# tudelft-iv/CCVPE

Measured on AMD Instinct MI355X. Metric: image-pairs/sec, higher is better.
Workload: dtype f32

## Files before the change

### ccvpe_amd/_lib.py

```python
import ctypes
import os
import subprocess

import torch

_HERE = os.path.dirname(os.path.abspath(__file__))
LIB_PATH = os.environ.get("CCVPE_LIB") or os.path.join(_HERE, "libccvpe_hip.so")
CSRC_DIR = os.path.join(_HERE, "csrc")

c_float_p = ctypes.c_void_p
c_int = ctypes.c_int
c_float = ctypes.c_float
c_void_p = ctypes.c_void_p


class ConvDesc(ctypes.Structure):
    _fields_ = [
        ("src0", c_void_p), ("src1", c_void_p), ("gate", c_void_p), ("w", c_void_p),
        ("scale", c_void_p), ("shift", c_void_p), ("residual", c_void_p), ("dst", c_void_p),
        ("c0", c_int), ("ld0", c_int), ("c1", c_int), ("ld1", c_int),
        ("batch", c_int), ("in_h", c_int), ("in_w", c_int),
        ("kh", c_int), ("kw", c_int), ("stride", c_int), ("pad", c_int),
        ("n", c_int), ("kpad", c_int), ("ldd", c_int), ("ldres", c_int),
        ("act", c_int), ("out_mode", c_int),
# ... 35 lines not shown
    "ccvpe_tail512_f32": (c_int, [ctypes.POINTER(TailDesc), c_void_p]),
    "ccvpe_tail512_bf16": (c_int, [ctypes.POINTER(TailDesc), c_void_p]),
    "ccvpe_conv_igemm_f32": (c_int, [ctypes.POINTER(ConvDesc), c_void_p]),
    "ccvpe_conv_igemm_splitk_floats": (c_int, [ctypes.POINTER(ConvDesc), c_int]),
    "ccvpe_conv_igemm_route": (c_int, [ctypes.POINTER(ConvDesc), c_int, c_int]),
    "ccvpe_set_narrow_kernels": (c_int, [c_int]),
    "ccvpe_set_pw_ring_kernels": (c_int, [c_int]),
    "ccvpe_set_mbconv_plane_kernels": (c_int, [c_int]),
    "ccvpe_mbconv_front_route": (c_int, [c_int] * 8),
    "ccvpe_mbconv_band_plan": (c_int, [c_int] * 7),
    "ccvpe_conv3x3_variant": (c_int, [ctypes.POINTER(ConvDesc), c_int]),
    "ccvpe_set_match_mfma": (c_int, [c_int]),
    "ccvpe_set_pwn_kernels": (c_int, [c_int]),
    "ccvpe_conv3x3_wino_ok": (c_int, [ctypes.POINTER(ConvDesc)]),
    "ccvpe_conv3x3_wino_f32": (c_int, [ctypes.POINTER(ConvDesc), c_void_p]),
    "ccvpe_conv3x3_match1_ok": (c_int, [ctypes.POINTER(ConvDesc), c_int, c_int]),
    "ccvpe_conv3x3_match1_bf16": (c_int, [ctypes.POINTER(ConvDesc), c_int, c_void_p, c_int, c_int, c_int, c_int, c_int, c_void_p, c_void_p]),
    "ccvpe_conv_igemm_splitk_f32": (c_int, [ctypes.POINTER(ConvDesc), c_void_p, c_void_p]),
    "ccvpe_conv_igemm_splitk_bf16": (c_int, [ctypes.POINTER(ConvDesc), c_int, c_void_p, c_void_p]),
    "ccvpe_upconv3x3_f32": (c_int, [ctypes.POINTER(UpconvDesc), c_void_p]),
    "ccvpe_upconv3x3_bf16": (c_int, [ctypes.POINTER(UpconvDesc), c_void_p]),
    "ccvpe_upconv3x3_route": (c_int, [ctypes.POINTER(UpconvDesc), c_int]),
    "ccvpe_upconv3x3_s3_ok": (c_int, [ctypes.POINTER(UpconvDesc)]),
    "ccvpe_upconv3x3_s3_f32": (c_int, [ctypes.POINTER(UpconvDesc), c_void_p]),
    "ccvpe_upconv3x3_s3_form_ok": (c_int, [ctypes.POINTER(UpconvDesc), c_int]),
    "ccvpe_upconv3x3_s3_form_f32": (c_int, [ctypes.POINTER(UpconvDesc), c_int, c_void_p]),
    "ccvpe_set_s3_quad": (c_int, [c_int]),
    "ccvpe_stem_conv_f32": (c_int, [c_void_p] * 5 + [c_int] * 4 + [c_void_p]),
    "ccvpe_dwconv_nblk": (c_int, [c_int] * 4),
    "ccvpe_dwconv_f32": (c_int, [c_void_p] * 6 + [c_int] * 7 + [c_void_p]),
# ... 141 lines not shown
```

### ccvpe_amd/csrc/plan.hip

```cpp
#include <cstring>
#include <string>
#include <unordered_map>
#include <utility>
#include <vector>

#include "common.h"

namespace ccvpe {

enum : uint32_t { K_INT = 0, K_FLT = 1, K_NULL = 2, K_WEIGHTS = 3, K_WORKSPACE = 4, K_GRD = 5, K_SAT = 6, K_STREAM = 7, K_BLOB = 8 };

template <typename A> struct FromSlot {
  static A get(uint64_t v) { return (A)(int64_t)v; }
};
template <typename P> struct FromSlot<P*> {
  static P* get(uint64_t v) { return reinterpret_cast<P*>((uintptr_t)v); }
};
template <> struct FromSlot<float> {
  static float get(uint64_t v) { uint32_t b = (uint32_t)v; float f; std::memcpy(&f, &b, 4); return f; }
};
template <typename... A, size_t... I>
static int invoke_seq(int (*f)(A...), const uint64_t* v, std::index_sequence<I...>) { return f(FromSlot<A>::get(v[I])...); }
template <typename... A>
static int invoke(int (*f)(A...), const uint64_t* v, int n) {
  if (n != (int)sizeof...(A)) return fail(CCVPE_EINVAL, "plan: call has %d arguments, the entry point takes %d", n, (int)sizeof...(A));
  return invoke_seq(f, v, std::index_sequence_for<A...>{});
}
typedef int (*Invoker)(const uint64_t*, int);

#define CCVPE_REG(fn) {#fn, [](const uint64_t* v, int n) -> int { return invoke(fn, v, n); }}
static const std::unordered_map<std::string, Invoker>& registry() {
  static const std::unordered_map<std::string, Invoker> r = {
      CCVPE_REG(ccvpe_conv_igemm_f32), CCVPE_REG(ccvpe_conv_igemm_bf16), CCVPE_REG(ccvpe_conv_igemm_splitk_f32),
      CCVPE_REG(ccvpe_conv_igemm_splitk_bf16), CCVPE_REG(ccvpe_conv3x3_match1_bf16), CCVPE_REG(ccvpe_conv3x3_wino_f32),
      CCVPE_REG(ccvpe_upconv3x3_f32), CCVPE_REG(ccvpe_upconv3x3_bf16), CCVPE_REG(ccvpe_upconv3x3_s3_f32),
      CCVPE_REG(ccvpe_tail512_f32), CCVPE_REG(ccvpe_tail512_bf16), CCVPE_REG(ccvpe_stem_conv_f32), CCVPE_REG(ccvpe_stem_conv_bf16),
      CCVPE_REG(ccvpe_stem_dw_f32), CCVPE_REG(ccvpe_stem_dw_bf16),
      CCVPE_REG(ccvpe_dwconv_f32), CCVPE_REG(ccvpe_dwconv_bf16), CCVPE_REG(ccvpe_mbconv_front_f32), CCVPE_REG(ccvpe_mbconv_front_bf16),
      CCVPE_REG(ccvpe_se_gate_f32), CCVPE_REG(ccvpe_ground_descriptor_f32), CCVPE_REG(ccvpe_match_level_f32),
      CCVPE_REG(ccvpe_match_level_bf16), CCVPE_REG(ccvpe_head_conv3x3_f32), CCVPE_REG(ccvpe_head_conv3x3_bf16),
      CCVPE_REG(ccvpe_softmax_rows_f32), CCVPE_REG(ccvpe_softmax_apply_f32), CCVPE_REG(ccvpe_cast_bf16_f32), CCVPE_REG(ccvpe_eval_postprocess_f32),
  };
  return r;
}
#undef CCVPE_REG

struct Patch { uint32_t call, arg, kind; uint64_t off; };
struct BlobPatch { uint32_t blob, field, kind; uint64_t off; };
struct Call { Invoker fn; std::string name; uint32_t first, nargs, sid; int wait_on; };
// ... 245 lines not shown
```

### ccvpe_amd/csrc/upconv_s3.hip

```cpp
#include "conv_common.h"

namespace ccvpe {

struct UpS3Params {
  const float* src0;
  const float* src1;
  const void* w;
  const float* shift9;
  float* dst;
  int c0, ld0, c1, ld1;
  int H1, W1, batch;
  int N, Npad;
  int nb0, nb1, nst;
  int ldd, act;
  int tiles_n, tiles_total;
};

template <int MT, int NT, int WN, bool PAIR>
struct UpS3Geom {
  static constexpr int WM = 4 / WN;
  static constexpr int BM = 16 * MT * WM;
  static constexpr int BN = 16 * NT * WN;
  static constexpr int TH = BM / 16;
  static constexpr int HR = TH + 2, HCP = PAIR ? 26 : 18;
  static constexpr int ROW = 24;
  static constexpr int HALO_DW = HR * HCP * ROW, ASTG_DW = 2 * BM * ROW;
  static constexpr int U_DW = HALO_DW > ASTG_DW ? HALO_DW : ASTG_DW;
  static constexpr int W_INSTR = (BN * 6 + 63) / 64;
  static constexpr int WBUF_DW = W_INSTR * 256;
  static constexpr int LDS_BYTES = (U_DW + 2 * WBUF_DW) * 4;
};

__device__ __forceinline__ unsigned pk_bf16(float a, float b) {
  typedef __bf16 bf16x2_t __attribute__((ext_vector_type(2)));
  bf16x2_t v;
  v[0] = (__bf16)a;
  v[1] = (__bf16)b;
  return __builtin_bit_cast(unsigned, v);
}
__device__ __forceinline__ float bf_lo(unsigned p) { return __builtin_bit_cast(float, p << 16); }
__device__ __forceinline__ float bf_hi(unsigned p) { return __builtin_bit_cast(float, p & 0xffff0000u); }

typedef unsigned u32x2 __attribute__((ext_vector_type(2)));
__device__ __forceinline__ void split3(f32x4 v, u32x2& hi, u32x2& mid, u32x2& lo) {
#pragma unroll
  for (int h = 0; h < 2; ++h) {
    float a = v[2 * h], b = v[2 * h + 1];
    const unsigned ph = pk_bf16(a, b);
    a -= bf_lo(ph);
    b -= bf_hi(ph);
    const unsigned pm = pk_bf16(a, b);
    a -= bf_lo(pm);
    b -= bf_hi(pm);
    hi[h] = ph;
    mid[h] = pm;
    lo[h] = pk_bf16(a, b);
  }
}

template <int MT, int NT, int WN, bool PAIR>
__global__ __launch_bounds__(256, 2) void upconv_s3_kernel(const UpS3Params p) {
  using G = UpS3Geom<MT, NT, WN, PAIR>;
  constexpr int BM = G::BM, BN = G::BN, TH = G::TH, HR = G::HR, HCP = G::HCP, ROW = G::ROW;
  constexpr int HC = PAIR ? 20 : 18, HPX = HR * HC;
  constexpr int H_IT = (HPX * 4 + 255) / 256;
  constexpr int A_IT = BM / 64;
  constexpr int WQ = (G::W_INSTR + 3) / 4;

  extern __shared__ __attribute__((aligned(16))) float s3_sm[];
  float* Us = s3_sm;
  float* Ws = s3_sm + G::U_DW;

  const int tid = threadIdx.x;
// ... 37 lines not shown
      h_pix[it] = -1;
    }
  }
  f32x4 h_reg[H_IT];
  unsigned h_keep = 0;
  auto load_halo = [&](int chunk) {
    h_keep = 0;
#pragma unroll
    for (int it = 0; it < H_IT; ++it) {
      const int ch = chunk * 16 + h_sub[it] * 4;
      const bool ok = h_pix[it] >= 0 && ch < p.c0;
      h_reg[it] = *reinterpret_cast<const f32x4*>(reinterpret_cast<const char*>(p.src0) + (ok ? ((unsigned)h_pix[it] * (unsigned)ld0s + (unsigned)ch) * 4u : 0u));
      h_keep |= ok ? (1u << it) : 0u;
    }
  };
  auto store_planes = [&](float* at, f32x4 v) {
    u32x2 hi, mid, lo;
    split3(v, hi, mid, lo);
    *reinterpret_cast<u32x2*>(at) = hi;
    *reinterpret_cast<u32x2*>(at + 8) = mid;
    *reinterpret_cast<u32x2*>(at + 16) = lo;
  };
  auto store_halo = [&]() {
#pragma unroll
    for (int it = 0; it < H_IT; ++it)
      if (h_off[it] >= 0) store_planes(Us + h_off[it], keep_if(h_reg[it], (h_keep >> it) & 1u));
  };

  unsigned wvoff[WQ];
  {
    const int valid = min(BN, p.Npad - n0) * 6;
#pragma unroll
    for (int q = 0; q < WQ; ++q) wvoff[q] = (unsigned)min((wave + 4 * q) * 64 + lane, valid - 1) * 16u;
  }
  const unsigned ws_lds = (unsigned)(uintptr_t)(__attribute__((address_space(3))) float*)Ws;
  const size_t stage_bytes = (size_t)p.Npad * (ROW * 4);
  const char* wpar = reinterpret_cast<const char*>(p.w) + ((size_t)par * p.nst * p.Npad + n0) * (ROW * 4);
// ... 266 lines not shown
```

### ccvpe_amd/models.py

```python
import torch
import torch.nn as nn

from . import ops
from .synth import B0_BLOCKS, MODEL_SPECS, state_dict_spec

BN_EPS = 1e-3
SKIP_BLOCKS = (15, 10, 4, 2, 0)
MATCH_STRIDES = {"vigor": (64, 32, 16, 8, 4, 2),
                 "kitti": (128, 64, 32, 16, 8, 8),
                 "oxford": (64, 32, 16, 8, 4, 2)}


def window_offset(kind, channels, length):
    return int(channels / 2 - length / 2) if kind == "oxford" else 0


def _round_up(v, m):
    return (v + m - 1) // m * m


class _Holder(nn.Module):

    def forward(self, *a, **k):
        raise RuntimeError("parameter holder is not callable; use the owning CVM_* module")
# ... 32 lines not shown
    return _pad2(w.permute(0, 2, 3, 1).reshape(o, -1), dtype)


_WINO_G = ((1.0, 0.0, 0.0), (0.5, 0.5, 0.5), (0.5, -0.5, 0.5), (0.0, 0.0, 1.0))


def _pack_wino(w, dtype=torch.float32):
    if dtype != torch.float32:
        return None
    o, i = w.shape[0], w.shape[1]
    g = torch.tensor(_WINO_G, dtype=torch.float64, device=w.device)
    u = torch.einsum("ak,ockl,bl->oabc", g, w.to(torch.float64), g)
    out = torch.zeros((_round_up(o, 32), 4, 4, _round_up(i, 16)), dtype=torch.float64, device=w.device)
    out[:o, :, :, :i] = u
    return out.reshape(out.shape[0], -1).to(torch.float32).contiguous()


def _fold_bn(sd, p):
    scale = sd[p + ".weight"] / torch.sqrt(sd[p + ".running_var"] + BN_EPS)
    shift = sd[p + ".bias"] - sd[p + ".running_mean"] * scale
    return scale.contiguous(), shift.contiguous()


class _Obj(object):
    pass


def _pack_encoder(sd, p, dtype=torch.float32, fold_bn=True):
    fold = _fold_bn if fold_bn else (lambda _sd, _p: (None, None))
    e = _Obj()
# ... 37 lines not shown


OVERLAP_DECODERS_MAX_BATCH = 128


def _overlap_decoders(precision, batch=1):
    return _OVERLAP_ENV == "1" or (_OVERLAP_ENV == "auto" and precision == "bf16" and batch <= OVERLAP_DECODERS_MAX_BATCH)
FOLD_LEVELS = tuple(int(c) for c in __import__("os").environ.get("CCVPE_FOLD_LEVELS", "012345"))
FOLD_MIN_PIXELS = int(__import__("os").environ.get("CCVPE_FOLD_MIN_PIXELS", "2048"))
FUSE_TAIL = __import__("os").environ.get("CCVPE_FUSE_TAIL", "1") != "0"
SPLIT_TAIL = __import__("os").environ.get("CCVPE_SPLIT_TAIL", "1") != "0"
WINO = __import__("os").environ.get("CCVPE_WINO", "1") != "0"
SPLIT3 = __import__("os").environ.get("CCVPE_SPLIT3", "1") != "0"
SPLIT3_TAIL = SPLIT3 and __import__("os").environ.get("CCVPE_SPLIT3_TAIL", "1") != "0"
SPLIT3_MIN_OK = 2
PACK_GRAPH = __import__("os").environ.get("CCVPE_PACK_GRAPH", "1") != "0"
PACK_GATHER = __import__("os").environ.get("CCVPE_PACK_GATHER", "1") != "0"
FUSE_MATCH = __import__("os").environ.get("CCVPE_FUSE_MATCH", "1") != "0"
FUSE_STEM = __import__("os").environ.get("CCVPE_FUSE_STEM", "1") != "0"
EVAL_TWO_STREAMS = __import__("os").environ.get("CCVPE_EVAL_TWO_STREAMS", "1") != "0"


def _tail_split(precision, x, cout):
    if x.dtype != torch.float32:
        return 0
    if precision == "bf16":
        return 1 if SPLIT_TAIL and cout == 1 else 0
    return 2 if SPLIT3 and SPLIT3_TAIL else 0


# ... 136 lines not shown
        lv.c, lv.ldo, lv.up_n = c, ldo, 4 * dc_out
        lv.up_w, lv.up_b = _pack_deconv(sd["deconv%d.weight" % lvl], sd["deconv%d.bias" % lvl],
                                        [(0, 1, c), (c, 0, 1)], ldo, dtype)
        lv.c0, lv.c1 = dc_out, c_in - dc_out
        lv.n_a = c_out
        if fold and j in FOLD_LEVELS:
            lv.fw, lv.fshift = _pack_upconv(sd["deconv%d.weight" % lvl], sd["deconv%d.bias" % lvl],
                                            [(0, 1, c), (c, 0, 1)], ldo, sd["conv%d.0.weight" % lvl],
                                            sd["conv%d.0.bias" % lvl], dtype)
            lv.fw3 = _pack_upconv_s3(lv.fw, ldo, lv.c1, dtype if base_dtype == torch.float32 else None)
        lv.w_a = _pack_conv(sd["conv%d.0.weight" % lvl], dtype)
        lv.b_a = sd["conv%d.0.bias" % lvl].contiguous()
        if lvl != 1:
            lv.w_b = _pack_conv(sd["conv%d.2.weight" % lvl], dtype)
            lv.u_b = _pack_wino(sd["conv%d.2.weight" % lvl], base_dtype) if fold else None
            lv.n_b = c_out
        else:
            lv.w_b = sd["conv1.2.weight"].permute(0, 2, 3, 1).contiguous()
        lv.b_b = sd["conv%d.2.bias" % lvl].contiguous()
        pk.loc.append(lv)
        dtype = base_dtype
        dc_in, dc_out, c_in, c_out = spec["ori"][j]
        ov = _Obj()
        if j == 0:
            c6 = dc_in - n_rot
            ov.k = pk.loc[0].ldo
            ov.k_algo = dc_in
            ov.up_w, ov.up_b = _pack_deconv(sd["deconv6_ori.weight"], sd["deconv6_ori.bias"],
                                            [(0, n_rot, c6), (c6 + 1, 0, n_rot)], pk.loc[0].ldo, dtype)
        else:
# ... 2 lines not shown
                                            [(0, 0, dc_in)], dc_in, dtype)
        ov.up_n = 4 * dc_out
        ov.c0, ov.c1 = dc_out, c_in - dc_out
        if fold and j in FOLD_LEVELS:
            cmap = [(0, n_rot, c6), (c6 + 1, 0, n_rot)] if j == 0 else [(0, 0, dc_in)]
            ov.fw, ov.fshift = _pack_upconv(sd["deconv%d_ori.weight" % lvl], sd["deconv%d_ori.bias" % lvl], cmap,
                                            ov.k, sd["conv%d_ori.0.weight" % lvl], sd["conv%d_ori.0.bias" % lvl],
                                            dtype)
            ov.fw3 = _pack_upconv_s3(ov.fw, ov.k, ov.c1, dtype)
        ov.w_a = _pack_conv(sd["conv%d_ori.0.weight" % lvl], dtype)
        ov.b_a = sd["conv%d_ori.0.bias" % lvl].contiguous()
        ov.n_a = c_out
        if lvl != 1:
            ov.w_b = _pack_conv(sd["conv%d_ori.2.weight" % lvl], dtype)
            ov.u_b = _pack_wino(sd["conv%d_ori.2.weight" % lvl], dtype) if fold else None
            ov.n_b = c_out
        else:
            ov.w_b = sd["conv1_ori.2.weight"].permute(0, 2, 3, 1).contiguous()
        ov.b_b = sd["conv%d_ori.2.bias" % lvl].contiguous()
        pk.ori.append(ov)
    pk.bwd = _pack_backward(sd, kind, pk) if (not fold and base_dtype == torch.float32) else None
    return pk


def _run_encoder(e, img, circular, multiscale, dtype=torch.float32):
    blk0 = e.blocks[0]
    stem_fused = (FUSE_STEM and not blk0.expand and blk0.k == 3 and blk0.s == 1 and blk0.mid == 32
                  and ops.stem_dw_supported(img.shape[2], img.shape[3], circular) > 0)
    x = None if stem_fused else ops.stem_conv(img, e.stem_w, e.stem_scale, e.stem_shift, circular, out_dtype=dtype)
    feats = []
# ... 20 lines not shown
        if multiscale:
            feats.append(x)
    b, h, w, _ = x.shape
    f = ops.conv_igemm(x, 320, e.w_head, 1280, batch=b, in_h=h, in_w=w, scale=e.head_scale,
                       shift=e.head_shift, act=ops.ACT_SWISH)
    return f, feats


def _double_conv(lv, up, skip, batch, hw):
    y = ops.conv_igemm(up, lv.c0, lv.w_a, lv.n_a, batch=batch, in_h=hw, in_w=hw, kh=3, kw=3, pad=1,
                       src1=skip, c1=lv.c1, shift=lv.b_a, act=ops.ACT_RELU)
    return y


def _conv_b(lv, y, batch, hw, out_f32=False):
    if (WINO and lv.u_b is not None and
            ops.conv3x3_wino_ok(y, lv.n_a, lv.u_b, lv.n_b, batch=batch, in_h=hw, in_w=hw)):
        return ops.conv3x3_wino(y, lv.n_a, lv.u_b, lv.n_b, batch=batch, in_h=hw, in_w=hw, shift=lv.b_b)
    return ops.conv_igemm(y, lv.n_a, lv.w_b, lv.n_b, batch=batch, in_h=hw, in_w=hw, kh=3, kw=3, pad=1, shift=lv.b_b,
                          out_f32=out_f32)


def _upconv_a(lv, x, k, batch, hw, skip):
    fw3 = getattr(lv, "fw3", None)
    if (SPLIT3 and fw3 is not None and
            ops.upconv3x3_s3_ok(x, k, fw3, lv.n_a, batch=batch, h1=hw, w1=hw, src1=skip, c1=lv.c1) >= SPLIT3_MIN_OK):
        return ops.upconv3x3_s3(x, k, fw3, lv.fshift, lv.n_a, batch=batch, h1=hw, w1=hw, src1=skip, c1=lv.c1, act=ops.ACT_RELU)
    return ops.upconv3x3(x, k, lv.fw, lv.fshift, lv.n_a, batch=batch, h1=hw, w1=hw, src1=skip, c1=lv.c1, act=ops.ACT_RELU)


# ... 299 lines not shown
```

### ccvpe_amd/ops.py

```python
import ctypes

import torch

from . import _lib
from ._lib import ConvDesc, check

ACT_NONE, ACT_RELU, ACT_SWISH, ACT_RELU_MASK = 0, 1, 2, 3
SPLIT_K_CALLS = 0
SPLIT_K = __import__("os").environ.get("CCVPE_SPLIT_K", "1") == "1"
OUT_NHWC, OUT_DECONV2X = 0, 1

_recorder = None


def set_recorder(rec):
    global _recorder
    _recorder = rec


class LaunchRecorder(object):

    def __init__(self):
        self.items = []

# ... 218 lines not shown
        dst = _empty((batch, in_h, in_w, ldd), device=src0.device)
    elif ldd is None:
        ldd = dst.shape[-1]
    d = _wino_desc(src0, c0, u_packed, n, batch, in_h, in_w, shift, dst, ldd, ld0)
    rec = _recorder
    ev0 = rec.begin() if rec is not None else None
    check(lib.ccvpe_conv3x3_wino_f32(ctypes.byref(d), _stream()), "ccvpe_conv3x3_wino_f32")
    if rec is not None:
        m = batch * in_h * in_w
        flops = 2.0 * m * n * 9 * c0
        nbytes = 4.0 * (m * c0 + m * n + n * 9 * c0)
        rec.end("conv3x3_wino_f32_kernel<16x16,32>", "3x3 s1 M%d N%d K%d" % (m, n, 9 * c0), flops, nbytes, ev0)
    return dst


def upconv3x3(src0, c0, w_packed, shift9, n, *, batch, h1, w1, src1=None, c1=0, act=ACT_NONE, algo_flops=None, route_only=False):
    lib = _lib.load()
    dt = _act_dtype(src0)
    for t, nm in ((src0, "src0"), (src1, "src1"), (w_packed, "w")):
        _chk(t, nm, dt)
    _chk(shift9, "shift9")
    dst = _empty((batch, 2 * h1, 2 * w1, n), device=src0.device, dtype=dt)
    d = _lib.UpconvDesc()
    d.src0, d.src1, d.w, d.shift9, d.dst = _ptr(src0), _ptr(src1), _ptr(w_packed), _ptr(shift9), _ptr(dst)
    d.c0, d.ld0, d.c1, d.ld1 = c0, src0.shape[-1], c1, (src1.shape[-1] if src1 is not None else 0)
    d.batch, d.h1, d.w1 = batch, h1, w1
    d.n, d.kpad, d.ldd, d.act = n, w_packed.shape[-1], n, act
    if route_only:
        return upconv_route(d, dt != torch.float32)
    rec = _recorder
# ... 460 lines not shown
```

### ccvpe_amd/plan.py

```python
import ctypes
import struct
import weakref

import torch

from . import _lib, ops

K_INT, K_FLT, K_NULL, K_WEIGHTS, K_WORKSPACE, K_GRD, K_SAT, K_STREAM, K_BLOB = range(9)
ALIGN = 256

LAUNCHES = ("ccvpe_conv_igemm_f32", "ccvpe_conv_igemm_bf16", "ccvpe_conv_igemm_splitk_f32", "ccvpe_conv_igemm_splitk_bf16",
            "ccvpe_conv3x3_match1_bf16", "ccvpe_conv3x3_wino_f32",
            "ccvpe_upconv3x3_f32", "ccvpe_upconv3x3_bf16", "ccvpe_upconv3x3_s3_f32", "ccvpe_tail512_f32", "ccvpe_tail512_bf16", "ccvpe_stem_conv_f32",
            "ccvpe_stem_conv_bf16", "ccvpe_stem_dw_f32", "ccvpe_stem_dw_bf16", "ccvpe_dwconv_f32", "ccvpe_dwconv_bf16", "ccvpe_mbconv_front_f32", "ccvpe_mbconv_front_bf16",
            "ccvpe_se_gate_f32", "ccvpe_ground_descriptor_f32", "ccvpe_match_level_f32", "ccvpe_match_level_bf16",
            "ccvpe_head_conv3x3_f32", "ccvpe_head_conv3x3_bf16", "ccvpe_softmax_rows_f32", "ccvpe_softmax_apply_f32", "ccvpe_cast_bf16_f32",
            "ccvpe_eval_postprocess_f32")
QUERIES = ("ccvpe_tail512_partials", "ccvpe_conv3x3_match1_ok", "ccvpe_conv3x3_wino_ok", "ccvpe_upconv3x3_s3_ok", "ccvpe_conv_igemm_splitk_floats", "ccvpe_conv_igemm_route", "ccvpe_conv3x3_variant", "ccvpe_upconv3x3_route", "ccvpe_dwconv_nblk", "ccvpe_mbconv_front_nblk", "ccvpe_mbconv_front_route", "ccvpe_mbconv_band_plan", "ccvpe_stem_dw_nblk",
           "ccvpe_last_error", "ccvpe_abi_version")


class _Arena(object):

    def __init__(self, size):
        self.size, self.free, self.peak = size, [(0, size)], 0

    def alloc(self, nbytes):
        n = max(ALIGN, (nbytes + ALIGN - 1) // ALIGN * ALIGN)
        for i, (off, sz) in enumerate(self.free):
            if sz >= n:
                if sz == n:
                    del self.free[i]
                else:
# ... 338 lines not shown
```

### include/ccvpe_hip.h

```cpp
#ifndef CCVPE_HIP_H
#define CCVPE_HIP_H

#ifdef __cplusplus
extern "C" {
#endif

#define CCVPE_OK 0
#define CCVPE_EINVAL (-1)
#define CCVPE_ELAUNCH (-2)

#define CCVPE_ACT_NONE 0
#define CCVPE_ACT_RELU 1
#define CCVPE_ACT_SWISH 2
#define CCVPE_ACT_RELU_MASK 3

#define CCVPE_OUT_NHWC 0
#define CCVPE_OUT_DECONV2X 1

#define CCVPE_MAX_SHIFTS 48

const char* ccvpe_last_error(void);
int ccvpe_abi_version(void);

typedef struct ccvpe_conv_desc {
// ... 20 lines not shown
int ccvpe_conv_igemm_splitk_floats(const ccvpe_conv_desc* desc, int is_bf16);
#define CCVPE_ROUTE_IGEMM 0
#define CCVPE_ROUTE_PW_GEMM 1
#define CCVPE_ROUTE_CONV3X3 2
#define CCVPE_ROUTE_C3N 3
#define CCVPE_ROUTE_PW_RING 4
#define CCVPE_ROUTE_PWN 5
int ccvpe_conv_igemm_route(const ccvpe_conv_desc* desc, int is_bf16, int out_f32);
int ccvpe_conv3x3_variant(const ccvpe_conv_desc* desc, int is_bf16);
int ccvpe_set_narrow_kernels(int on);
int ccvpe_set_pw_ring_kernels(int on);
int ccvpe_set_pwn_kernels(int on);
int ccvpe_set_mbconv_plane_kernels(int mode);
int ccvpe_conv3x3_wino_ok(const ccvpe_conv_desc* desc);
int ccvpe_conv3x3_wino_f32(const ccvpe_conv_desc* desc, void* stream);
int ccvpe_conv3x3_match1_ok(const ccvpe_conv_desc* desc, int out_f32, int L);
int ccvpe_conv3x3_match1_bf16(const ccvpe_conv_desc* desc, int out_f32, const float* g, int ldg, int L, int shift, int stride,
                              int window_offset, float* scores, void* stream);
int ccvpe_conv_igemm_splitk_f32(const ccvpe_conv_desc* desc, float* scratch, void* stream);

typedef struct ccvpe_upconv_desc {
  const void* src0;
  const void* src1;
  const void* w;
  const float* shift9;
  void* dst;
  int c0, ld0, c1, ld1;
  int batch, h1, w1;
  int n, kpad, ldd;
  int act;
// ... 233 lines not shown
```

Measured before the change: 2742.

## Add Winograd 3x3 conv kernel using three-way bf16 split on MFMA

```diff
diff --git a/ccvpe_amd/_lib.py b/ccvpe_amd/_lib.py
--- a/ccvpe_amd/_lib.py
+++ b/ccvpe_amd/_lib.py
@@ -73,6 +73,8 @@
     "ccvpe_set_pwn_kernels": (c_int, [c_int]),
     "ccvpe_conv3x3_wino_ok": (c_int, [ctypes.POINTER(ConvDesc)]),
     "ccvpe_conv3x3_wino_f32": (c_int, [ctypes.POINTER(ConvDesc), c_void_p]),
+    "ccvpe_conv3x3_wino_s3_ok": (c_int, [ctypes.POINTER(ConvDesc)]),
+    "ccvpe_conv3x3_wino_s3_f32": (c_int, [ctypes.POINTER(ConvDesc), c_void_p]),
     "ccvpe_conv3x3_match1_ok": (c_int, [ctypes.POINTER(ConvDesc), c_int, c_int]),
     "ccvpe_conv3x3_match1_bf16": (c_int, [ctypes.POINTER(ConvDesc), c_int, c_void_p, c_int, c_int, c_int, c_int, c_int, c_void_p, c_void_p]),
     "ccvpe_conv_igemm_splitk_f32": (c_int, [ctypes.POINTER(ConvDesc), c_void_p, c_void_p]),
diff --git a/ccvpe_amd/csrc/conv3x3_wino_s3.hip b/ccvpe_amd/csrc/conv3x3_wino_s3.hip
--- /dev/null
+++ b/ccvpe_amd/csrc/conv3x3_wino_s3.hip
@@ -0,0 +1,317 @@
+#include "conv_common.h"
+#include "split3.h"
+
+namespace ccvpe {
+
+struct WinoS3Params {
+  const float* src0;
+  const void* w;
+  const float* shift;
+  float* dst;
+  int c0, ld0;
+  int H, W;
+  int N, Npad;
+  int ldd;
+  int tiles_x, tiles_y, tiles_n, tiles_total;
+};
+
+static constexpr int WS_NTHR = 512;
+static constexpr int WS_BN = 64;
+static constexpr int WS_TILES = 64;
+static constexpr int WS_HC = 18, WS_HPX = 18 * WS_HC;
+static constexpr int WS_HALO_DW = WS_HPX * LDS_LD;
+static constexpr int WS_PANEL_DW = 4 * WS_TILES * S3_ROW;
+static constexpr int WS_LDS = (2 * WS_HALO_DW + 4 * WS_PANEL_DW) * 4;
+static_assert(WS_LDS <= 160 * 1024, "conv3x3_wino_s3_kernel: LDS of one CU");
+
+__global__ __launch_bounds__(WS_NTHR) void conv3x3_wino_s3_kernel(const WinoS3Params p) {
+  constexpr int H_IT = (WS_HPX * 4 + WS_NTHR - 1) / WS_NTHR;
+  extern __shared__ __attribute__((aligned(16))) float ws_sm[];
+  float* Vs = ws_sm;
+  float* Us = Vs + 2 * WS_PANEL_DW;
+  float* Hs = Us + 2 * WS_PANEL_DW;
+
+  const int tid = threadIdx.x;
+  const int lane = tid & 63;
+  const int wave = sgpr(tid >> 6);
+
+  const int tile = xcd_tile(blockIdx.x, p.tiles_total);
+  const int tn = tile % p.tiles_n;
+  const int ts = tile / p.tiles_n;
+  const int tx = ts % p.tiles_x;
+  const int ty = (ts / p.tiles_x) % p.tiles_y;
+  const int b = ts / (p.tiles_x * p.tiles_y);
+  const int y0 = ty * 16, x0 = tx * 16;
+  const int n0 = tn * WS_BN;
+  const int ctot = p.c0;
+  const int nchunks = (ctot + 15) / 16;
+  const int nstages = nchunks * 4;
+
+  int h_off[H_IT], h_pix[H_IT];
+  const int h_sub = tid & 3;
+#pragma unroll
+  for (int it = 0; it < H_IT; ++it) {
+    const int idx = tid + WS_NTHR * it;
+    const int px = idx >> 2;
+    if (px < WS_HPX) {
+      const int hy = px / WS_HC, hx = px - hy * WS_HC;
+      const int iy = y0 - 1 + hy, ix = x0 - 1 + hx;
+      h_off[it] = px * LDS_LD + h_sub * 4;
+      h_pix[it] = ((unsigned)iy < (unsigned)p.H && (unsigned)ix < (unsigned)p.W) ? (b * p.H + iy) * p.W + ix : -1;
+    } else {
+      h_off[it] = -1;
+      h_pix[it] = -1;
+    }
+  }
+  f32x4 h_reg[H_IT];
+  int h_chunk = 0;
+  const int ld0s = sgpr(p.ld0);
+  auto load_halo = [&](int chunk) {
+    h_chunk = chunk;
+#pragma unroll
+    for (int it = 0; it < H_IT; ++it) {
+      const int ch = chunk * 16 + h_sub * 4;
+      const bool ok = h_pix[it] >= 0 && ch < ctot;
+      const size_t off = ok ? (size_t)h_pix[it] * ld0s + ch : 0;
+      h_reg[it] = *reinterpret_cast<const f32x4*>(p.src0 + off);
+    }
+  };
+  auto store_halo = [&](int hbuf) {
+#pragma unroll
+    for (int it = 0; it < H_IT; ++it)
+      if (h_off[it] >= 0)
+        *reinterpret_cast<f32x4*>(Hs + hbuf * WS_HALO_DW + h_off[it]) =
+            keep_if(h_reg[it], h_pix[it] >= 0 && h_chunk * 16 + h_sub * 4 < ctot);
+  };
+
+  const unsigned us_lds = (unsigned)(uintptr_t)(__attribute__((address_space(3))) float*)Us;
+  const size_t comp_bytes = (size_t)p.Npad * (S3_ROW * 4);
+  const char* wbase = reinterpret_cast<const char*>(p.w) + (size_t)n0 * (S3_ROW * 4);
+  const unsigned wvoff = (unsigned)lane * 16u;
+  auto load_u = [&](int s, int dbuf) {
+#pragma unroll
+    for (int q = 0; q < 3; ++q) {
+      const int i = wave * 3 + q;
+      const int c = i / 6, piece = i - 6 * c;
+      const char* sbase = wbase + (size_t)(s * 4 + c) * comp_bytes + piece * 1024;
+      const unsigned lds = __builtin_amdgcn_readfirstlane(us_lds + (unsigned)(dbuf * WS_PANEL_DW * 4 + i * 1024));
+      asm volatile("s_mov_b32 m0, %0\n\tglobal_load_lds_dwordx4 %1, %2" ::"s"(lds), "v"(wvoff), "s"(sbase) : "memory", "m0");
+    }
+  };
+  auto dma_wait = [&]() { asm volatile("s_waitcnt vmcnt(0)" ::: "memory"); };
+
+  const int v_sub = tid & 3;
+  const int v_tile = (tid >> 2) & 63;
+  const int v_half = wave >> 2;
+  const int v_src = ((2 * (v_tile >> 3)) * WS_HC + 2 * (v_tile & 7) + v_half) * LDS_LD + v_sub * 4;
+  const int v_dst = ((2 * v_half) * WS_TILES + v_tile) * S3_ROW + v_sub * 2;
+  f32x4 t_da[3], t_db[3], t_va, t_vb;
+  auto tr_read = [&](auto rtag, int hbuf) {
+    constexpr int R = decltype(rtag)::value;
+    constexpr int RA = R == 0 ? 0 : (R == 2 ? 2 : 1);
+    constexpr int RB = R == 0 ? 2 : (R == 1 ? 2 : (R == 2 ? 1 : 3));
+    const float* hs = Hs + hbuf * WS_HALO_DW + v_src;
+#pragma unroll
+    for (int x = 0; x < 3; ++x) {
+      t_da[x] = *reinterpret_cast<const f32x4*>(hs + (RA * WS_HC + x) * LDS_LD);
+      t_db[x] = *reinterpret_cast<const f32x4*>(hs + (RB * WS_HC + x) * LDS_LD);
+    }
+  };
+  auto tr_math = [&](auto rtag) {
+    constexpr int R = decltype(rtag)::value;
+    f32x4 t[3];
+#pragma unroll
+    for (int x = 0; x < 3; ++x) t[x] = R == 1 ? t_da[x] + t_db[x] : t_da[x] - t_db[x];
+    if (v_half == 0) {
+      t_va = t[0] - t[2];
+      t_vb = t[1] + t[2];
+    } else {
+      t_va = t[1] - t[0];
+      t_vb = t[0] - t[2];
+    }
+  };
+  auto tr_store = [&](int which, int vbuf) {
+    float* vd = Vs + vbuf * WS_PANEL_DW + v_dst;
+    if (which == 0) s3_store_planes(vd, t_va);
+    else s3_store_planes(vd + WS_TILES * S3_ROW, t_vb);
+  };
+  auto transform = [&](auto rtag, int hbuf, int vbuf) {
+    tr_read(rtag, hbuf);
+    tr_math(rtag);
+    tr_store(0, vbuf);
+    tr_store(1, vbuf);
+  };
+
+  f32x4 acc[16][2];
+#pragma unroll
+  for (int x = 0; x < 16; ++x)
+#pragma unroll
+    for (int j = 0; j < 2; ++j) acc[x][j] = (f32x4){0.f, 0.f, 0.f, 0.f};
+
+  const int frow = lane & 15;
+  const int g4 = lane >> 4;
+  const int fk = g4 * 4;
+  const int tb = wave >> 1, cp = wave & 1;
+  const int vfrag = (tb * 16 + frow) * S3_ROW;
+  const int ufrag = (cp * 32 + frow) * S3_ROW;
+  const int v1off = vfrag + s3_frag_hi_hi(g4), v2off = vfrag + s3_frag_mid_mid(g4), v3off = vfrag + s3_frag_hi_lo(g4);
+  const int u1off = ufrag + s3_frag_hi_mid(g4), u2off = ufrag + s3_frag_lo_hi(g4);
+
+  load_halo(0);
+  load_u(0, 0);
+  store_halo(0);
+  __syncthreads();
+  transform(std::integral_constant<int, 0>{}, 0, 0);
+  dma_wait();
+  __syncthreads();
+
+  int chunk = 0;
+  auto stage = [&](int s, auto rtag) {
+    constexpr int R = decltype(rtag)::value;
+    const bool more = s + 1 < nstages;
+    const bool next_chunk = chunk + 1 < nchunks;
+    if (R == 0 && next_chunk) load_halo(chunk + 1);
+    if (more) load_u(s + 1, (R + 1) & 1);
+    if (R == 2 && next_chunk) store_halo((chunk + 1) & 1);
+    const bool do_tr = R < 3 || more;
+    const int tr_hbuf = (R < 3 ? chunk : chunk + 1) & 1;
+    constexpr auto ntag = std::integral_constant<int, (R + 1) & 3>{};
+    const float* vb = Vs + (R & 1) * WS_PANEL_DW;
+    const float* ub = Us + (R & 1) * WS_PANEL_DW;
+#pragma unroll
+    for (int c = 0; c < 4; ++c) {
+      const float* vc = vb + c * (WS_TILES * S3_ROW);
+      const float* uc = ub + c * (WS_BN * S3_ROW);
+      const f32x4 v1 = *reinterpret_cast<const f32x4*>(vc + v1off);
+      const f32x4 v2 = *reinterpret_cast<const f32x4*>(vc + v2off);
+      const f32x4 v3 = *reinterpret_cast<const f32x4*>(vc + v3off);
+      f32x4 u1[2], u2[2];
+#pragma unroll
+      for (int j = 0; j < 2; ++j) {
+        u1[j] = *reinterpret_cast<const f32x4*>(uc + j * 16 * S3_ROW + u1off);
+        u2[j] = *reinterpret_cast<const f32x4*>(uc + j * 16 * S3_ROW + u2off);
+      }
+      if (c == 0 && do_tr) tr_read(ntag, tr_hbuf);
+#pragma unroll
+      for (int j = 0; j < 2; ++j) acc[R * 4 + c][j] = mfma_stage<bf16_t>(u1[j], v1, acc[R * 4 + c][j]);
+#pragma unroll
+      for (int j = 0; j < 2; ++j) acc[R * 4 + c][j] = mfma_stage<bf16_t>(u1[j], v2, acc[R * 4 + c][j]);
+#pragma unroll
+      for (int j = 0; j < 2; ++j) acc[R * 4 + c][j] = mfma_stage<bf16_t>(u2[j], v3, acc[R * 4 + c][j]);
+      if (do_tr) {
+        if (c == 0) tr_math(ntag);
+        if (c == 1) tr_store(0, (R + 1) & 1);
+        if (c == 2) tr_store(1, (R + 1) & 1);
+      }
+    }
+    dma_wait();
+    __syncthreads();
+  };
+  for (int s = 0; s < nstages; s += 4, ++chunk) {
+    stage(s, std::integral_constant<int, 0>{});
+    stage(s + 1, std::integral_constant<int, 1>{});
+    stage(s + 2, std::integral_constant<int, 2>{});
+    stage(s + 3, std::integral_constant<int, 3>{});
+  }
+
+  const int etile = tb * 16 + frow;
+  const int oy = y0 + 2 * (etile >> 3), ox = x0 + 2 * (etile & 7);
+  if (oy >= p.H || ox >= p.W) return;
+  const size_t m00 = (size_t)(b * p.H + oy) * p.W + ox;
+#pragma unroll
+  for (int j = 0; j < 2; ++j) {
+    const int n = n0 + (cp * 2 + j) * 16 + fk;
+    if (n >= p.N) continue;
+    f32x4 y[2][2];
+#pragma unroll
+    for (int r = 0; r < 4; ++r) {
+      float m[4][4];
+#pragma unroll
+      for (int x = 0; x < 16; ++x) m[x >> 2][x & 3] = acc[x][j][r];
+      float q0[4], q1[4];
+#pragma unroll
+      for (int c = 0; c < 4; ++c) {
+        q0[c] = m[0][c] + m[1][c] + m[2][c];
+        q1[c] = m[1][c] - m[2][c] - m[3][c];
+      }
+      const float bias = (p.shift && n + r < p.N) ? p.shift[n + r] : 0.0f;
+      y[0][0][r] = q0[0] + q0[1] + q0[2] + bias;
+      y[0][1][r] = q0[1] - q0[2] - q0[3] + bias;
+      y[1][0][r] = q1[0] + q1[1] + q1[2] + bias;
+      y[1][1][r] = q1[1] - q1[2] - q1[3] + bias;
+    }
+#pragma unroll
+    for (int dy = 0; dy < 2; ++dy)
+#pragma unroll
+      for (int dx = 0; dx < 2; ++dx) {
+        const size_t o = (m00 + (size_t)dy * p.W + dx) * p.ldd + n;
+        if (n + 3 < p.N) {
+          *reinterpret_cast<f32x4*>(p.dst + o) = y[dy][dx];
+        } else {
+#pragma unroll
+          for (int r = 0; r < 4; ++r)
+            if (n + r < p.N) p.dst[o + r] = y[dy][dx][r];
+        }
+      }
+  }
+}
+
+static int ws_round_up(int v, int m) { return (v + m - 1) / m * m; }
+
+static const char* wino_s3_refusal(const ccvpe_conv_desc* d) {
+  if (!d) return "null desc";
+  if (d->kh != 3 || d->kw != 3 || d->stride != 1 || d->pad != 1 || d->out_mode != CCVPE_OUT_NHWC) return "3x3 / stride 1 / pad 1 / NHWC only";
+  if (d->c1 != 0 || d->src1 || d->gate || d->scale || d->residual || d->act != CCVPE_ACT_NONE)
+    return "one source, bias only (no gate, scale, residual or activation)";
+  if (d->batch <= 0 || d->in_h <= 0 || d->in_w <= 0 || d->in_h % 2 || d->in_w % 2) return "H and W must be even";
+  if (d->c0 < 32 || d->c0 % 4 || d->ld0 < d->c0 || d->ld0 % 4) return "c0 >= 32, c0 and ld0 multiples of 4";
+  if (d->n <= 0 || d->ldd < d->n || d->ldd % 4) return "ldd >= n, ldd multiple of 4";
+  if (d->kpad != 16 * 48 * ((d->c0 + 15) / 16)) return "kpad must be 768 * ceil(c0 / 16) (the three-plane pack of models._pack_wino_s3)";
+  if ((long)d->batch * d->in_h * d->in_w > 0x7fffffffL) return "too many pixels";
+  if ((double)ws_round_up(d->n, WS_BN) * d->kpad * 2.0 >= 4294967296.0) return "U larger than 4 GB";
+  return nullptr;
+}
+
+}
+
+using namespace ccvpe;
+
+static constexpr long WINO_S3_MIN_WGS = 640;
+static constexpr int WINO_S3_MIN_N = 1;
+static long wino_s3_workgroups(const ccvpe_conv_desc* d) {
+  return (long)((d->in_w + 15) / 16) * ((d->in_h + 15) / 16) * d->batch * (ws_round_up(d->n, WS_BN) / WS_BN);
+}
+static int wino_s3_rule(const ccvpe_conv_desc* d) {
+  return (wino_s3_workgroups(d) >= WINO_S3_MIN_WGS && d->n >= WINO_S3_MIN_N) ? 2 : 1;
+}
+
+extern "C" int ccvpe_conv3x3_wino_s3_ok(const ccvpe_conv_desc* d) {
+  if (wino_s3_refusal(d)) return 0;
+  return wino_s3_rule(d);
+}
+
+extern "C" int ccvpe_conv3x3_wino_s3_f32(const ccvpe_conv_desc* d, void* stream) {
+  if (const char* why = wino_s3_refusal(d)) return fail(CCVPE_EINVAL, "conv3x3_wino_s3: %s", why);
+  if (!d->src0 || !d->w || !d->dst) return fail(CCVPE_EINVAL, "conv3x3_wino_s3: null pointer");
+  if (!aligned16(d->src0) || !aligned16(d->w) || !aligned16(d->dst)) return fail(CCVPE_EINVAL, "conv3x3_wino_s3: pointers must be 16-byte aligned");
+  WinoS3Params p{};
+  p.src0 = reinterpret_cast<const float*>(d->src0); p.w = d->w; p.shift = d->shift; p.dst = reinterpret_cast<float*>(d->dst);
+  p.c0 = d->c0; p.ld0 = d->ld0;
+  p.H = d->in_h; p.W = d->in_w;
+  p.N = d->n; p.Npad = ws_round_up(d->n, WS_BN);
+  p.ldd = d->ldd;
+  p.tiles_x = (p.W + 15) / 16;
+  p.tiles_y = (p.H + 15) / 16;
+  p.tiles_n = p.Npad / WS_BN;
+  const long total = (long)p.tiles_x * p.tiles_y * d->batch * p.tiles_n;
+  if (total > 0x7fffffffL) return fail(CCVPE_EINVAL, "conv3x3_wino_s3: grid too large");
+  p.tiles_total = (int)total;
+  static bool attr_set = false;
+  if (!attr_set) {
+    hipError_t e = hipFuncSetAttribute((const void*)conv3x3_wino_s3_kernel, hipFuncAttributeMaxDynamicSharedMemorySize, WS_LDS);
+    if (e != hipSuccess) return fail(CCVPE_ELAUNCH, "conv3x3_wino_s3: set smem attr: %s", hipGetErrorString(e));
+    attr_set = true;
+  }
+  hipLaunchKernelGGL(conv3x3_wino_s3_kernel, dim3(p.tiles_total), dim3(WS_NTHR), WS_LDS, (hipStream_t)stream, p);
+  return check_launch("conv3x3_wino_s3_kernel");
+}
diff --git a/ccvpe_amd/csrc/plan.hip b/ccvpe_amd/csrc/plan.hip
--- a/ccvpe_amd/csrc/plan.hip
+++ b/ccvpe_amd/csrc/plan.hip
@@ -33,6 +33,7 @@
   static const std::unordered_map<std::string, Invoker> r = {
       CCVPE_REG(ccvpe_conv_igemm_f32), CCVPE_REG(ccvpe_conv_igemm_bf16), CCVPE_REG(ccvpe_conv_igemm_splitk_f32),
       CCVPE_REG(ccvpe_conv_igemm_splitk_bf16), CCVPE_REG(ccvpe_conv3x3_match1_bf16), CCVPE_REG(ccvpe_conv3x3_wino_f32),
+      CCVPE_REG(ccvpe_conv3x3_wino_s3_f32),
       CCVPE_REG(ccvpe_upconv3x3_f32), CCVPE_REG(ccvpe_upconv3x3_bf16), CCVPE_REG(ccvpe_upconv3x3_s3_f32),
       CCVPE_REG(ccvpe_tail512_f32), CCVPE_REG(ccvpe_tail512_bf16), CCVPE_REG(ccvpe_stem_conv_f32), CCVPE_REG(ccvpe_stem_conv_bf16),
       CCVPE_REG(ccvpe_stem_dw_f32), CCVPE_REG(ccvpe_stem_dw_bf16),
diff --git a/ccvpe_amd/csrc/split3.h b/ccvpe_amd/csrc/split3.h
--- /dev/null
+++ b/ccvpe_amd/csrc/split3.h
@@ -0,0 +1,48 @@
+#pragma once
+#include "conv_common.h"
+
+namespace ccvpe {
+
+constexpr int S3_ROW = 24;
+
+__device__ __forceinline__ unsigned pk_bf16(float a, float b) {
+  typedef __bf16 bf16x2_t __attribute__((ext_vector_type(2)));
+  bf16x2_t v;
+  v[0] = (__bf16)a;
+  v[1] = (__bf16)b;
+  return __builtin_bit_cast(unsigned, v);
+}
+__device__ __forceinline__ float bf_lo(unsigned p) { return __builtin_bit_cast(float, p << 16); }
+__device__ __forceinline__ float bf_hi(unsigned p) { return __builtin_bit_cast(float, p & 0xffff0000u); }
+
+typedef unsigned u32x2 __attribute__((ext_vector_type(2)));
+__device__ __forceinline__ void split3(f32x4 v, u32x2& hi, u32x2& mid, u32x2& lo) {
+#pragma unroll
+  for (int h = 0; h < 2; ++h) {
+    float a = v[2 * h], b = v[2 * h + 1];
+    const unsigned ph = pk_bf16(a, b);
+    a -= bf_lo(ph);
+    b -= bf_hi(ph);
+    const unsigned pm = pk_bf16(a, b);
+    a -= bf_lo(pm);
+    b -= bf_hi(pm);
+    hi[h] = ph;
+    mid[h] = pm;
+    lo[h] = pk_bf16(a, b);
+  }
+}
+__device__ __forceinline__ void s3_store_planes(float* row_piece, f32x4 v) {
+  u32x2 hi, mid, lo;
+  split3(v, hi, mid, lo);
+  *reinterpret_cast<u32x2*>(row_piece) = hi;
+  *reinterpret_cast<u32x2*>(row_piece + 8) = mid;
+  *reinterpret_cast<u32x2*>(row_piece + 16) = lo;
+}
+
+__device__ __forceinline__ int s3_frag_hi_mid(int g4) { return 4 * g4; }
+__device__ __forceinline__ int s3_frag_lo_hi(int g4) { return g4 < 2 ? 16 + 4 * g4 : 4 * g4 - 8; }
+__device__ __forceinline__ int s3_frag_hi_hi(int g4) { return 4 * (g4 & 1); }
+__device__ __forceinline__ int s3_frag_mid_mid(int g4) { return 8 + 4 * (g4 & 1); }
+__device__ __forceinline__ int s3_frag_hi_lo(int g4) { return g4 < 2 ? 4 * g4 : 4 * g4 + 8; }
+
+}
diff --git a/ccvpe_amd/csrc/upconv_s3.hip b/ccvpe_amd/csrc/upconv_s3.hip
--- a/ccvpe_amd/csrc/upconv_s3.hip
+++ b/ccvpe_amd/csrc/upconv_s3.hip
@@ -1,4 +1,5 @@
 #include "conv_common.h"
+#include "split3.h"
 
 namespace ccvpe {
 
@@ -24,39 +25,13 @@
   static constexpr int TH = BM / 16;
   static constexpr int HR = TH + 2, HCP = PAIR ? 26 : 18;
   static constexpr int ROW = 24;
+  static_assert(ROW == S3_ROW, "the row of split3.h");
   static constexpr int HALO_DW = HR * HCP * ROW, ASTG_DW = 2 * BM * ROW;
   static constexpr int U_DW = HALO_DW > ASTG_DW ? HALO_DW : ASTG_DW;
   static constexpr int W_INSTR = (BN * 6 + 63) / 64;
   static constexpr int WBUF_DW = W_INSTR * 256;
   static constexpr int LDS_BYTES = (U_DW + 2 * WBUF_DW) * 4;
 };
-
-__device__ __forceinline__ unsigned pk_bf16(float a, float b) {
-  typedef __bf16 bf16x2_t __attribute__((ext_vector_type(2)));
-  bf16x2_t v;
-  v[0] = (__bf16)a;
-  v[1] = (__bf16)b;
-  return __builtin_bit_cast(unsigned, v);
-}
-__device__ __forceinline__ float bf_lo(unsigned p) { return __builtin_bit_cast(float, p << 16); }
-__device__ __forceinline__ float bf_hi(unsigned p) { return __builtin_bit_cast(float, p & 0xffff0000u); }
-
-typedef unsigned u32x2 __attribute__((ext_vector_type(2)));
-__device__ __forceinline__ void split3(f32x4 v, u32x2& hi, u32x2& mid, u32x2& lo) {
-#pragma unroll
-  for (int h = 0; h < 2; ++h) {
-    float a = v[2 * h], b = v[2 * h + 1];
-    const unsigned ph = pk_bf16(a, b);
-    a -= bf_lo(ph);
-    b -= bf_hi(ph);
-    const unsigned pm = pk_bf16(a, b);
-    a -= bf_lo(pm);
-    b -= bf_hi(pm);
-    hi[h] = ph;
-    mid[h] = pm;
-    lo[h] = pk_bf16(a, b);
-  }
-}
 
 template <int MT, int NT, int WN, bool PAIR>
 __global__ __launch_bounds__(256, 2) void upconv_s3_kernel(const UpS3Params p) {
@@ -124,13 +99,7 @@
       h_keep |= ok ? (1u << it) : 0u;
     }
   };
-  auto store_planes = [&](float* at, f32x4 v) {
-    u32x2 hi, mid, lo;
-    split3(v, hi, mid, lo);
-    *reinterpret_cast<u32x2*>(at) = hi;
-    *reinterpret_cast<u32x2*>(at + 8) = mid;
-    *reinterpret_cast<u32x2*>(at + 16) = lo;
-  };
+  auto store_planes = [&](float* at, f32x4 v) { s3_store_planes(at, v); };
   auto store_halo = [&]() {
 #pragma unroll
     for (int it = 0; it < H_IT; ++it)
diff --git a/ccvpe_amd/models.py b/ccvpe_amd/models.py
--- a/ccvpe_amd/models.py
+++ b/ccvpe_amd/models.py
@@ -70,6 +70,17 @@
     out = torch.zeros((_round_up(o, 32), 4, 4, _round_up(i, 16)), dtype=torch.float64, device=w.device)
     out[:o, :, :, :i] = u
     return out.reshape(out.shape[0], -1).to(torch.float32).contiguous()
+
+
+def _pack_wino_s3(w, dtype=torch.float32):
+    if dtype != torch.float32:
+        return None
+    o, i = w.shape[0], w.shape[1]
+    nch = _round_up(i, 16) // 16
+    u = _pack_wino(w).reshape(-1, 16, nch, 16)[:o]
+    out = u.new_zeros((nch, 16, _round_up(o, 64), 16))
+    out[:, :, :o] = u.permute(2, 1, 0, 3)
+    return torch.cat(_split3_bf16(out), -1).reshape(nch * 16, out.shape[2], 48).contiguous()
 
 
 def _fold_bn(sd, p):
@@ -137,6 +148,7 @@
 SPLIT3 = __import__("os").environ.get("CCVPE_SPLIT3", "1") != "0"
 SPLIT3_TAIL = SPLIT3 and __import__("os").environ.get("CCVPE_SPLIT3_TAIL", "1") != "0"
 SPLIT3_MIN_OK = 2
+WINO_S3 = WINO and __import__("os").environ.get("CCVPE_WINO_S3", "1") != "0"
 PACK_GRAPH = __import__("os").environ.get("CCVPE_PACK_GRAPH", "1") != "0"
 PACK_GATHER = __import__("os").environ.get("CCVPE_PACK_GATHER", "1") != "0"
 FUSE_MATCH = __import__("os").environ.get("CCVPE_FUSE_MATCH", "1") != "0"
@@ -303,6 +315,7 @@
         if lvl != 1:
             lv.w_b = _pack_conv(sd["conv%d.2.weight" % lvl], dtype)
             lv.u_b = _pack_wino(sd["conv%d.2.weight" % lvl], base_dtype) if fold else None
+            lv.u_b3 = _pack_wino_s3(sd["conv%d.2.weight" % lvl], base_dtype) if fold and WINO_S3 else None
             lv.n_b = c_out
         else:
             lv.w_b = sd["conv1.2.weight"].permute(0, 2, 3, 1).contiguous()
@@ -335,6 +348,7 @@
         if lvl != 1:
             ov.w_b = _pack_conv(sd["conv%d_ori.2.weight" % lvl], dtype)
             ov.u_b = _pack_wino(sd["conv%d_ori.2.weight" % lvl], dtype) if fold else None
+            ov.u_b3 = _pack_wino_s3(sd["conv%d_ori.2.weight" % lvl], dtype) if fold and WINO_S3 else None
             ov.n_b = c_out
         else:
             ov.w_b = sd["conv1_ori.2.weight"].permute(0, 2, 3, 1).contiguous()
@@ -385,6 +399,10 @@
 
 
 def _conv_b(lv, y, batch, hw, out_f32=False):
+    u_b3 = getattr(lv, "u_b3", None)
+    if (WINO and WINO_S3 and u_b3 is not None and
+            ops.conv3x3_wino_s3_ok(y, lv.n_a, u_b3, lv.n_b, batch=batch, in_h=hw, in_w=hw) >= SPLIT3_MIN_OK):
+        return ops.conv3x3_wino_s3(y, lv.n_a, u_b3, lv.n_b, batch=batch, in_h=hw, in_w=hw, shift=lv.b_b)
     if (WINO and lv.u_b is not None and
             ops.conv3x3_wino_ok(y, lv.n_a, lv.u_b, lv.n_b, batch=batch, in_h=hw, in_w=hw)):
         return ops.conv3x3_wino(y, lv.n_a, lv.u_b, lv.n_b, batch=batch, in_h=hw, in_w=hw, shift=lv.b_b)
diff --git a/ccvpe_amd/ops.py b/ccvpe_amd/ops.py
--- a/ccvpe_amd/ops.py
+++ b/ccvpe_amd/ops.py
@@ -256,6 +256,48 @@
     return dst
 
 
+def _wino_s3_desc(src0, c0, u3_packed, n, batch, in_h, in_w, shift, dst, ldd, ld0):
+    d = _wino_desc(src0, c0, u3_packed, n, batch, in_h, in_w, shift, dst, ldd, ld0)
+    d.kpad = u3_packed.shape[0] * u3_packed.shape[2]
+    return d
+
+
+def conv3x3_wino_s3_ok(src0, c0, u3_packed, n, *, batch, in_h, in_w, ldd=None, ld0=None):
+    if u3_packed is None or src0.dtype != torch.float32:
+        return 0
+    if u3_packed.dtype != torch.bfloat16 or tuple(u3_packed.shape) != ((c0 + 15) // 16 * 16, (n + 63) // 64 * 64, 48):
+        return 0
+    ld0 = ld0 if ld0 is not None else src0.shape[-1]
+    d = _wino_s3_desc(src0, c0, u3_packed, n, batch, in_h, in_w, None, None, ldd if ldd is not None else n, ld0)
+    return int(_lib.load().ccvpe_conv3x3_wino_s3_ok(ctypes.byref(d)))
+
+
+def conv3x3_wino_s3(src0, c0, u3_packed, n, *, batch, in_h, in_w, shift=None, dst=None, ldd=None, ld0=None):
+    lib = _lib.load()
+    for t, nm in ((src0, "src0"), (shift, "shift"), (dst, "dst")):
+        _chk(t, nm)
+    _chk(u3_packed, "w", torch.bfloat16)
+    ld0 = ld0 if ld0 is not None else src0.shape[-1]
+    if not conv3x3_wino_s3_ok(src0, c0, u3_packed, n, batch=batch, in_h=in_h, in_w=in_w, ldd=ldd if ldd is not None else (dst.shape[-1] if dst is not None else n), ld0=ld0):
+        raise _lib.CcvpeError("conv3x3_wino_s3: layer not served (c0 %d, n %d, %d x %d, pack %s)"
+                              % (c0, n, in_h, in_w, tuple(u3_packed.shape)))
+    if dst is None:
+        ldd = ldd if ldd is not None else n
+        dst = _empty((batch, in_h, in_w, ldd), device=src0.device)
+    elif ldd is None:
+        ldd = dst.shape[-1]
+    d = _wino_s3_desc(src0, c0, u3_packed, n, batch, in_h, in_w, shift, dst, ldd, ld0)
+    rec = _recorder
+    ev0 = rec.begin() if rec is not None else None
+    check(lib.ccvpe_conv3x3_wino_s3_f32(ctypes.byref(d), _stream()), "ccvpe_conv3x3_wino_s3_f32")
+    if rec is not None:
+        m = batch * in_h * in_w
+        flops = 2.0 * m * n * 9 * c0
+        nbytes = 4.0 * (m * c0 + m * n + n * 9 * c0)
+        rec.end("conv3x3_wino_s3_kernel<64x64>", "3x3 s1 M%d N%d K%d" % (m, n, 9 * c0), flops, nbytes, ev0)
+    return dst
+
+
 def upconv3x3(src0, c0, w_packed, shift9, n, *, batch, h1, w1, src1=None, c1=0, act=ACT_NONE, algo_flops=None, route_only=False):
     lib = _lib.load()
     dt = _act_dtype(src0)
diff --git a/ccvpe_amd/plan.py b/ccvpe_amd/plan.py
--- a/ccvpe_amd/plan.py
+++ b/ccvpe_amd/plan.py
@@ -10,13 +10,13 @@
 ALIGN = 256
 
 LAUNCHES = ("ccvpe_conv_igemm_f32", "ccvpe_conv_igemm_bf16", "ccvpe_conv_igemm_splitk_f32", "ccvpe_conv_igemm_splitk_bf16",
-            "ccvpe_conv3x3_match1_bf16", "ccvpe_conv3x3_wino_f32",
+            "ccvpe_conv3x3_match1_bf16", "ccvpe_conv3x3_wino_f32", "ccvpe_conv3x3_wino_s3_f32",
             "ccvpe_upconv3x3_f32", "ccvpe_upconv3x3_bf16", "ccvpe_upconv3x3_s3_f32", "ccvpe_tail512_f32", "ccvpe_tail512_bf16", "ccvpe_stem_conv_f32",
             "ccvpe_stem_conv_bf16", "ccvpe_stem_dw_f32", "ccvpe_stem_dw_bf16", "ccvpe_dwconv_f32", "ccvpe_dwconv_bf16", "ccvpe_mbconv_front_f32", "ccvpe_mbconv_front_bf16",
             "ccvpe_se_gate_f32", "ccvpe_ground_descriptor_f32", "ccvpe_match_level_f32", "ccvpe_match_level_bf16",
             "ccvpe_head_conv3x3_f32", "ccvpe_head_conv3x3_bf16", "ccvpe_softmax_rows_f32", "ccvpe_softmax_apply_f32", "ccvpe_cast_bf16_f32",
             "ccvpe_eval_postprocess_f32")
-QUERIES = ("ccvpe_tail512_partials", "ccvpe_conv3x3_match1_ok", "ccvpe_conv3x3_wino_ok", "ccvpe_upconv3x3_s3_ok", "ccvpe_conv_igemm_splitk_floats", "ccvpe_conv_igemm_route", "ccvpe_conv3x3_variant", "ccvpe_upconv3x3_route", "ccvpe_dwconv_nblk", "ccvpe_mbconv_front_nblk", "ccvpe_mbconv_front_route", "ccvpe_mbconv_band_plan", "ccvpe_stem_dw_nblk",
+QUERIES = ("ccvpe_tail512_partials", "ccvpe_conv3x3_match1_ok", "ccvpe_conv3x3_wino_ok", "ccvpe_conv3x3_wino_s3_ok", "ccvpe_upconv3x3_s3_ok", "ccvpe_conv_igemm_splitk_floats", "ccvpe_conv_igemm_route", "ccvpe_conv3x3_variant", "ccvpe_upconv3x3_route", "ccvpe_dwconv_nblk", "ccvpe_mbconv_front_nblk", "ccvpe_mbconv_front_route", "ccvpe_mbconv_band_plan", "ccvpe_stem_dw_nblk",
            "ccvpe_last_error", "ccvpe_abi_version")
 
 
diff --git a/include/ccvpe_hip.h b/include/ccvpe_hip.h
--- a/include/ccvpe_hip.h
+++ b/include/ccvpe_hip.h
@@ -58,6 +58,8 @@
 int ccvpe_set_mbconv_plane_kernels(int mode);
 int ccvpe_conv3x3_wino_ok(const ccvpe_conv_desc* desc);
 int ccvpe_conv3x3_wino_f32(const ccvpe_conv_desc* desc, void* stream);
+int ccvpe_conv3x3_wino_s3_ok(const ccvpe_conv_desc* desc);
+int ccvpe_conv3x3_wino_s3_f32(const ccvpe_conv_desc* desc, void* stream);
 int ccvpe_conv3x3_match1_ok(const ccvpe_conv_desc* desc, int out_f32, int L);
 int ccvpe_conv3x3_match1_bf16(const ccvpe_conv_desc* desc, int out_f32, const float* g, int ldg, int L, int shift, int stride,
                               int window_offset, float* scores, void* stream);
```

Measured after the change: 2660. -3.0%, worse.
